# starreeze/drin

Measured on AMD Instinct MI355X. Metric: mention x candidate pairs scored/sec, higher is better.
Workload: dtype bf16x3; 1 GPU; wikimel-shaped scoring forward: 100-cand (+1 answer slot), D=768, R=2048, L=128, P=49, T=64 token-level entity text; parallelism=dp1 (mentions sharded, no collective)

## Files before the change

drin_amd/csrc/entity_cache.hip:

```cpp
#include <string.h>

#include "fused.h"
#include "internal.h"
#include "layout.h"
#include "row_ops.h"

namespace drin {

static inline bool cache_mixed(const drin_config& c) { return c.cache_format == DRIN_CACHE_MIXED_F16; }
static inline size_t cache_row_floats(const drin_config& c) {
  const size_t D = (size_t)c.embed_dim, R = (size_t)c.image_dim;
  return cache_mixed(c) ? 4 * D + R / 2 + 4 : 5 * D + R + 4;
}
constexpr int64_t kCacheSlab = 262144;

struct CacheBuildArgs {
  const float* entity_text;
  const int64_t* entity_mask;
  const float* entity_object;
  const float* entity_object_score;
  float* xt;
  float* cache;
  int64_t ldc, rows;
  int D4, R4, T, Ke;
// ... 410 lines not shown
  }
  __syncthreads();
  float* out1 = a.c_part + (b * a.chunks + blockIdx.x) * (int64_t)(2 * D + 4);
  float* out2 = a.s2_part + (b * a.chunks + blockIdx.x) * (int64_t)(2 * D);
  auto waves_sum = [&](int i) {
    return ((ld4(l_acc + i * 4) + ld4(l_acc + 3 * D + i * 4)) + ld4(l_acc + 6 * D + i * 4)) + ld4(l_acc + 9 * D + i * 4);
  };
  for (int i = threadIdx.x; i < 2 * D4; i += 256) {
    st4(out1 + i * 4, waves_sum(i));
    st4(out2 + i * 4, i < D4 ? waves_sum(2 * D4 + i) : make_float4(0.f, 0.f, 0.f, 0.f));
  }
  if (threadIdx.x < 4) {
    const float* s4 = l_small + 8 + threadIdx.x;
    out1[2 * D + threadIdx.x] = ((s4[0] + s4[4]) + s4[8]) + s4[12];
  }
}

__global__ void __launch_bounds__(256) k_mention_layer1_cached(const float* __restrict__ part, const float* __restrict__ hm,
                                                               int ldhm, const float* __restrict__ cb_t,
                                                               const float* __restrict__ cb_i, const float* __restrict__ b_h,
                                                               float* __restrict__ out, int B, int D, int chunks, float inv_n) {
  const int64_t b = blockIdx.y;
  const int d = blockIdx.x * 256 + threadIdx.x;
  if (d >= D) return;
  const int width = 2 * D + 4;
  float at = 0.f, ai = 0.f, s0 = 0.f, s1 = 0.f, s2 = 0.f, s3 = 0.f;
  for (int c = 0; c < chunks; ++c) {
    const float* p = part + (b * chunks + c) * (int64_t)width;
    at += p[d];
    ai += p[D + d];
    s0 += p[2 * D];
    s1 += p[2 * D + 1];
    s2 += p[2 * D + 2];
    s3 += p[2 * D + 3];
  }
  const float bh = b_h[d], wt = cb_t[d] - bh, wi = cb_i[d] - bh;
  out[b * D + d] = (at + s0 * wt + s1 * wi) * inv_n + hm[b * ldhm + d] + bh;
  out[((int64_t)B + b) * D + d] = (ai + s2 * wt + s3 * wi) * inv_n + hm[((int64_t)B + b) * ldhm + d] + bh;
}

static int cached_chunk_candidates(const drin_config& c) {
  const bool exact = c.embed_dim == 768 && c.image_dim == 2048 && vertex_act(&c) == DRIN_ACT_GELU;
  if (!exact) return 16;
  return c.batch >= 2048 ? 128 : 64;
}

struct CachedLayout {
  size_t span_mean, mimg, vm0, hmfu, e1m, c_part, s2_part, vm1, hm2, agg2, mt2, et1, p_et1, h2, splitk, splitk_floats, total;
  int chunks;
  void build(const drin_config& c) {
    const size_t B = c.batch, N = c.num_candidates, D = c.embed_dim, R = c.image_dim, M = B * N;
    chunks = (int)((N + cached_chunk_candidates(c) - 1) / cached_chunk_candidates(c));
    size_t off = 0;
// ... 276 lines not shown
      DRIN_TRY((launch_cached_pairs_t<3, 8, true, false, true>(a, st)));
    else
      DRIN_TRY((launch_cached_pairs_t<3, 8, false, false, true>(a, st)));
  } else if (a.act_v != DRIN_ACT_GELU && a.D4 <= 64 && a.R4 <= 64)
    DRIN_TRY((launch_cached_pairs_t<1, 1, false, true>(a, st)));
  else if (a.act_v != DRIN_ACT_GELU)
    DRIN_TRY((launch_cached_pairs_t<3, 8, false, true>(a, st)));
  else if (a.D4 <= 64 && a.R4 <= 64)
    DRIN_TRY((launch_cached_pairs_t<1, 1, false>(a, st)));
  else if (a.D4 == 192 && a.R4 == 512)
    DRIN_TRY((launch_cached_pairs_t<3, 8, true>(a, st)));
  else
    DRIN_TRY((launch_cached_pairs_t<3, 8, false>(a, st)));

  float* vm1 = ws + L.vm1;
  {
    KernelTimer timer(DRIN_KC_GCN, st);
    hipLaunchKernelGGL(k_mention_layer1_cached, dim3((unsigned)cdiv(D, 256), (unsigned)B), dim3(256), 0, st, ws + L.c_part,
                       hmfu, 2 * D, pb + P.cb_t, pb + P.cb_i, L1.b_h, vm1, B, D, L.chunks, 1.0f / (float)N);
    DRIN_CHECK_LAUNCH("k_mention_layer1_cached");
  }
  DRIN_TRY(run_folded_mention_finish(cfg, params, pb, P, weight_planes, vm1, ws + L.hm2, msk, st));
  return run_folded_tail(cfg, params, pb, P, L.chunks, ws + L.s2_part, vm1, ws + L.agg2, ws + L.mt2, ws + L.hm2, ws + L.e1m, ws + L.h2,
                         planes ? nullptr : ws + L.et1, planes ? e1_hi : nullptr, weight_planes, msk, {}, scores, st);
}

}
```

drin_amd/csrc/fused.h:

```cpp
#pragma once
#include <hip/hip_runtime.h>
#include <stddef.h>
#include <stdint.h>
#include <string.h>

#include "../../include/drin_hip.h"
#include "layout.h"

namespace drin {

struct Prepared {
  size_t wcat1, bcat1, ecat, etmp, k_t, k_i, c_txt, c_img, cb_t, cb_i, total;
  size_t p_ctxt, p_cimg, p_wh2;
  size_t p_wmt, p_wmi, p_wcat1, p_ecat, p_wet, p_wei, p_wh1;
  size_t p_cimg_f16;
  size_t cimg_f16_scale;
  void build(const drin_config& c) {
    const size_t D = c.embed_dim, R = c.image_dim;
    size_t off = 0;
    auto take = [&off](size_t n) {
      const size_t o = off;
      off += (n + 63) & ~(size_t)63;
      return o;
    };
    wcat1 = take(2 * D * D);
    bcat1 = take(2 * D);
    ecat = take(D * (D + R));
    etmp = take(D * (D + R));
    k_t = take(D);
    k_i = take(D);
    c_txt = take(D * D);
    c_img = take(D * R);
    cb_t = take(D);
    cb_i = take(D);
    p_ctxt = take(D * D);
    p_cimg = take(D * R);
    p_wh2 = take(D * D);
    p_wmt = take(D * D);
    p_wmi = take(D * R);
    p_wcat1 = take(2 * D * D);
    p_ecat = take(D * (D + R));
    p_wet = take(D * D);
    p_wei = take(D * R);
    p_wh1 = take(D * D);
    p_cimg_f16 = take(D * R / 2 + 2);
    cimg_f16_scale = take(2);
    total = off;
  }
};

int fused_supported(const drin_config* c);
int cached_chunks_per_mention(const drin_config& c);

struct StreamArgs {
  const void* entity_text;
  const int64_t* entity_mask;
  const void* entity_image;
  const void* entity_object;
  const float* entity_object_score;
// ... 6 lines not shown
  const void* mobj;
  const float* mscore;
  const float* fu;
  const float* q;
  const float* k_t;
  const float* k_i;
  float* xt_out;
  void* xt_hi;
  void* xt_lo;
  void* xi_hi;
  void* xi_lo;
  float* xi_scale;
  void* xi_f16;
  float* e0m;
  float* e1m;
  float* s_part;
  float* s_text;
  float* s_img;
  float* sig;
  int B, N, D4, R4, T, Km, Ke, chunks, ldq, ldfu, dynamic, bf16_features;
  int act_e;
  float mask[4];
  float cos_eps, miei_eps, clip;
};

struct PairArgs {
  const float* h_text;
  const float* h_image;
  const float* hm;
  const float* c_t;
  const float* c_i;
  const float* gamma;
  const float* beta;
  const float* e0m;
  const float* e1m;
  float* et1;
  void* et1_hi;
  void* et1_lo;
  float* s2_part;
  int B, N, D4, chunks, ldhm;
  int act_v;
  float ln_eps;
};

struct FinalArgs {
  const float* h2;
  const float* hm2;
  const float* b_h2;
  const float* gamma;
  const float* beta;
  const float* e1m;
  const float* mt2;
  float* scores;
  int B, N, D4, chunks;
// ... 10 lines not shown
}
template <class Args>
void set_vertex_fields(Args& a, const drin_config& c) {
  a.ln_eps = c.layer_norm_eps, a.act_v = vertex_act(&c);
}
template <class Args>
void set_edge_fields(Args& a, const drin_config& c) {
  a.R4 = c.image_dim / 4;
  a.Km = c.mention_objects;
  a.dynamic = c.dynamic_edges != 0;
  a.act_e = edge_act(&c);
  for (int k = 0; k < 4; ++k) a.mask[k] = c.edge_enabled[k];
  a.cos_eps = c.cosine_eps, a.miei_eps = c.miei_eps, a.clip = c.clip_scale;
}

size_t entity_stream_lds_bytes(const StreamArgs& a);
int launch_entity_stream(const StreamArgs& a, hipStream_t st);
int launch_reduce_stream_partials(const float* part, float* s_text, float* s_img, float* sig, int B, int D, int R,
                                  int chunks, hipStream_t st);
int launch_mention_input1(const float* T, const float* T2, const float* sig, const float* b_et, const float* b_ei,
                          const float* v0, float* out, int B, int D, int N, hipStream_t st);
int launch_pair_layer1(const PairArgs& a, hipStream_t st);
int launch_mention_input2(const float* part, const float* mt1, float* out, int B, int D, int N, int chunks,
                          hipStream_t st);
int launch_pair_final(const FinalArgs& a, hipStream_t st);

struct GemmScratch {
  float* p = nullptr;
  size_t floats = 0;
};
int run_folded_head(const drin_config* cfg, const drin_batch* b, const drin_params* params, const float* prepared, const Prepared& P,
                    bool weight_planes, float* span_mean, float* mimg, float* vm0, float* hmfu, GemmScratch mention_sk, hipStream_t st);
int run_folded_mention_finish(const drin_config* cfg, const drin_params* params, const float* prepared, const Prepared& P,
                              bool weight_planes, float* vm1, float* hm2, GemmScratch mention_sk, hipStream_t st);
int run_folded_tail(const drin_config* cfg, const drin_params* params, const float* prepared, const Prepared& P, int chunks,
                    const float* s2_part, const float* vm1, float* agg2, float* mt2, const float* hm2, const float* e1m, float* h2,
// ... 4 lines not shown
```

drin_amd/csrc/fused_forward.hip:

```cpp
#include <string.h>

#include "fused.h"
#include "internal.h"
#include "layout.h"

namespace drin {

constexpr int kMixedMinCandidates = 64;

struct FusedLayout {
  size_t span_mean, mimg, vm0, hmfu, q, e0m, e1m, xt, s_part, s_text, s_img, sig, tm, tm2, agg1, vm1, hm2, h_text, h_image,
      et1, s2_part, agg2, mt2, p_xt, p_xi, p_et1, xi_scale, splitk, splitk_floats, pair_splitk, pair_splitk_floats, total;
  int chunks;
  void build(const drin_config& c) {
    const size_t B = c.batch, N = c.num_candidates, D = c.embed_dim, R = c.image_dim, M = B * N;
    chunks = (int)(B >= 2048 ? (N + 127) / 128 : B >= 1024 ? (N + 47) / 48 : (N + 15) / 16);
    size_t off = 0;
    auto take = [&off](size_t n) {
      const size_t o = off;
      off += (n + 63) & ~(size_t)63;
      return o;
    };
    span_mean = take(B * D);
    mimg = take(B * R);
    vm0 = take(2 * B * D);
    hmfu = take(2 * B * 2 * D);
    q = take(2 * B * (D + R));
    e0m = take(4 * M);
    e1m = take(4 * M);
    xt = take(c.entity_tokens > 0 ? M * D : 0);
    s_part = take(B * chunks * (2 * D + 2 * R + 4));
    s_text = take(2 * B * D);
    s_img = take(2 * B * R);
    sig = take(4 * B);
    tm = take(2 * B * D);
    tm2 = take(2 * B * D);
    agg1 = take(2 * B * D);
    vm1 = take(2 * B * D);
    hm2 = take(2 * B * D);
    h_text = take(M * D);
    h_image = take(M * D);
    et1 = take(M * D);
    s2_part = take(B * chunks * 2 * D);
    agg2 = take(B * D);
    mt2 = take(B * D);
    const bool planes = c.precision == DRIN_PREC_BF16X3 || c.precision == DRIN_PREC_BF16X3_ALL || c.precision == DRIN_PREC_BF16X3_IF16;
    p_xt = take(planes ? M * D : 0);
    p_xi = take(!planes ? 0 : c.num_entities > 0 ? M * R : c.precision == DRIN_PREC_BF16X3_IF16 ? M * R / 2 : 0);
    p_et1 = take(planes ? M * D : 0);
    xi_scale = take(c.precision == DRIN_PREC_BF16X3_IF16 ? M : 0);
    splitk_floats = 2 * B <= 512 ? 8 * 2 * B * (D + R) : 0;
    if (planes && splitk_floats < (size_t)192 * 65536) splitk_floats = (size_t)192 * 65536;
// ... 120 lines not shown
  DRIN_TRY(launch_gemm_nn(L1.w_h, D, params->w_entity_text, D, pb + P.c_txt, D, D, D, D, false, F32, st));
  DRIN_TRY(launch_gemm_nn(L1.w_h, D, params->w_entity_image, R, pb + P.c_img, R, D, R, D, false, F32, st));
  DRIN_TRY(launch_gemm_nt(params->b_entity_text, D, L1.w_h, D, L1.b_h, pb + P.cb_t, D, 1, D, D, false, F32, st));
  DRIN_TRY(launch_gemm_nt(params->b_entity_image, D, L1.w_h, D, L1.b_h, pb + P.cb_i, D, 1, D, D, false, F32, st));
  {
    const size_t dd = (size_t)D * D, dr = (size_t)D * R;
    __bf16* q = reinterpret_cast<__bf16*>(pb + P.p_ctxt);
    DRIN_TRY(launch_split_planes(pb + P.c_txt, q, q + dd, dd, st));
    q = reinterpret_cast<__bf16*>(pb + P.p_cimg);
    DRIN_TRY(launch_split_planes(pb + P.c_img, q, q + dr, dr, st));
    DRIN_TRY(launch_to_f16_scaled(pb + P.c_img, pb + P.p_cimg_f16, (int64_t)dr, pb + P.cimg_f16_scale, st));
    q = reinterpret_cast<__bf16*>(pb + P.p_wh2);
    DRIN_TRY(launch_split_planes(params->layer[1].w_h, q, q + dd, dd, st));
    struct { size_t off; const float* w; size_t n; } extra[] = {
        {P.p_wmt, params->w_mention_text, dd},  {P.p_wmi, params->w_mention_image, dr},
        {P.p_wcat1, pb + P.wcat1, 2 * dd},      {P.p_ecat, pb + P.ecat, dd + dr},
        {P.p_wet, params->w_entity_text, dd},   {P.p_wei, params->w_entity_image, dr},
        {P.p_wh1, L1.w_h, dd}};
    for (const auto& e : extra) {
      q = reinterpret_cast<__bf16*>(pb + e.off);
      DRIN_TRY(launch_split_planes(e.w, q, q + e.n, e.n, st));
    }
  }
  return DRIN_OK;
}

}

namespace drin {

static int folded_precision(const drin_config* c) { return c->precision == DRIN_PREC_BF16X3_IF16 ? (int)DRIN_PREC_BF16X3 : c->precision; }

int run_folded_head(const drin_config* cfg, const drin_batch* b, const drin_params* params, const float* pb, const Prepared& P,
// ... 131 lines not shown
  sa.k_t = pb + P.k_t;
  sa.k_i = pb + P.k_i;
  sa.xt_out = planes ? nullptr : ws + L.xt;
  if (planes) {
    sa.xt_hi = xt_hi;
    sa.xt_lo = xt_exact ? nullptr : xt_hi + MD;
    if (xi_planes) {
      sa.xi_hi = xi_hi;
      sa.xi_lo = bf16_feat ? nullptr : xi_hi + MR;
    }
  }
  sa.xi_scale = if16 ? ws + L.xi_scale : nullptr;
  sa.xi_f16 = if16 ? static_cast<void*>(xi_hi) : nullptr;
  sa.e0m = ws + L.e0m;
  sa.e1m = ws + L.e1m;
  sa.s_part = ws + L.s_part;
  sa.T = cfg->entity_tokens;
  sa.Ke = cfg->entity_objects;
  sa.chunks = L.chunks;
  sa.bf16_features = bf16_feat ? 1 : 0;
  sa.s_text = ws + L.s_text;
  sa.s_img = ws + L.s_img;
  sa.sig = ws + L.sig;
  DRIN_TRY(launch_entity_stream(sa, st));
  if (L.chunks > 1)
    DRIN_TRY(launch_reduce_stream_partials(ws + L.s_part, ws + L.s_text, ws + L.s_img, ws + L.sig, B, D, R, L.chunks, st));
  DRIN_TRY(launch_gemm_nt_pair({ws + L.s_text, params->w_entity_text, nullptr, ws + L.tm, D, D, D, 2 * (int64_t)B, D, D, wp(P.p_wet)},
                               {ws + L.s_img, params->w_entity_image, nullptr, ws + L.tm2, R, R, D, 2 * (int64_t)B, D, R,
                                wp(P.p_wei)},
                               prec, st, msk.p, msk.floats));
  DRIN_TRY(launch_mention_input1(ws + L.tm, ws + L.tm2, ws + L.sig, params->b_entity_text, params->b_entity_image, vm0, ws + L.agg1, B, D, N, st));
  float* vm1 = ws + L.vm1;
  DRIN_TRY(launch_gemm_nt(ws + L.agg1, D, L1.w_h, D, L1.b_h, vm1, D, 2 * (int64_t)B, D, D, false, prec, st, msk.p, msk.floats, wp(P.p_wh1)));
  DRIN_TRY(run_folded_mention_finish(cfg, params, pb, P, planes, vm1, ws + L.hm2, msk, st));
  const GemmScratch psk = L.pair_splitk_floats ? GemmScratch{ws + L.pair_splitk, L.pair_splitk_floats} : msk;
  if (planes) {
    const __bf16* ct = reinterpret_cast<const __bf16*>(pb + P.p_ctxt);
    const __bf16* ci = reinterpret_cast<const __bf16*>(pb + P.p_cimg);
    DRIN_TRY(launch_gemm_x3_planes(xt_hi, xt_exact ? nullptr : xt_hi + MD, D, ct, ct + (size_t)D * D, D, nullptr, ws + L.h_text, D, M, D,
                                   D, st, psk.p, psk.floats));
    if (if16)
      DRIN_TRY(launch_gemm_f16_planes(xi_hi, R, pb + P.p_cimg_f16, R, ws + L.xi_scale, pb + P.cimg_f16_scale, ws + L.h_image, D, M, D, R,
                                      st, psk.p, psk.floats));
    else if (xi_planes)
      DRIN_TRY(launch_gemm_x3_planes(xi_hi, bf16_feat ? nullptr : xi_hi + MR, R, ci, ci + (size_t)D * R, R, nullptr, ws + L.h_image, D, M,
                                     D, R, st, psk.p, psk.floats));
    else if (bf16_feat)
      DRIN_TRY(launch_gemm_x3_planes(b->entity_image, nullptr, R, ci, ci + (size_t)D * R, R, nullptr, ws + L.h_image, D, M, D, R, st, psk.p,
                                     psk.floats));
// ... 11 lines not shown
  pa.h_image = ws + L.h_image;
  pa.hm = hmfu;
  pa.ldhm = 2 * D;
  pa.c_t = pb + P.cb_t;
  pa.c_i = pb + P.cb_i;
  pa.gamma = L1.ln_weight;
  pa.beta = L1.ln_bias;
  pa.e0m = ws + L.e0m;
  pa.e1m = ws + L.e1m;
  pa.et1 = planes ? nullptr : ws + L.et1;
  if (planes) {
    pa.et1_hi = e1_hi;
    pa.et1_lo = e1_hi + MD;
  }
  pa.s2_part = ws + L.s2_part;
  pa.chunks = L.chunks;
  DRIN_TRY(launch_pair_layer1(pa, st));
  return run_folded_tail(cfg, params, pb, P, L.chunks, ws + L.s2_part, vm1, ws + L.agg2, ws + L.mt2, ws + L.hm2, ws + L.e1m, ws + L.h_text,
                         planes ? nullptr : ws + L.et1, planes ? e1_hi : nullptr, planes, msk, psk, scores, st);
}

}

extern "C" {

int32_t drin_workgroups_per_mention(const drin_config* cfg, int32_t cached) {
  if (validate_config(cfg) != DRIN_OK || fused_supported(cfg) != DRIN_OK) return 0;
  if (cached) return cached_chunks_per_mention(*cfg);
  FusedLayout L;
  L.build(*cfg);
  return L.chunks;
}
// ... 56 lines not shown
```

drin_amd/csrc/fused_kernels.hip:

```cpp
#include "device_utils.h"
#include "fused.h"
#include "internal.h"
#include "row_ops.h"

namespace drin {

template <int DV, int RV, bool TOKENS, bool EXACT, typename FT, bool XSCALE = false>
__global__ void __launch_bounds__(256, 2) k_entity_stream(const StreamArgs a) {
  extern __shared__ __attribute__((aligned(16))) float lds[];
  const FT* const f_text = static_cast<const FT*>(a.entity_text);
  const FT* const f_image = static_cast<const FT*>(a.entity_image);
  const FT* const f_object = static_cast<const FT*>(a.entity_object);
  const FT* const f_mobj = static_cast<const FT*>(a.mobj);
  const int D4 = EXACT ? DV * 64 : a.D4, R4 = EXACT ? RV * 64 : a.R4, D = D4 * 4, R = R4 * 4;
  constexpr bool RP = sizeof(FT) == 2 && (RV % 2) == 0;
  auto load_r = [&](const FT* row) -> Row<RV> {
    if constexpr (RP)
      return load_row_stream_pair<RV>(row, (int)(threadIdx.x & 63), R4);
    else
      return load_row_stream<RV>(row, (int)(threadIdx.x & 63), R4);
  };
  float* l_mobj = lds;
  float* l_q = l_mobj + a.Km * R;
  float* l_red = l_q + 2 * R;
  float* l_mt = l_red + 2 * D + 2 * R;
  float* l_small = l_mt + 3 * D;
  const int wave = threadIdx.x >> 6, lane = threadIdx.x & 63;
  const int64_t b = blockIdx.y;
  const int per = (a.N + a.chunks - 1) / a.chunks;
  const int n_begin = blockIdx.x * per, n_end = min(a.N, n_begin + per);
  const bool dyn = a.dynamic != 0;

  for (int i = threadIdx.x; i < a.Km * R4; i += 256) st4(l_mobj + i * 4, ld4(f_mobj + (b * a.Km) * R + i * 4));
  for (int i = threadIdx.x; i < D4; i += 256) st4(l_mt + i * 4, ld4(a.span_mean + b * D + i * 4));
  if (dyn) {
    for (int i = threadIdx.x; i < 2 * R4; i += 256) {
      const int which = i / R4, c4 = i - which * R4;
      st4(l_q + i * 4, ld4(a.q + ((int64_t)which * a.B + b) * a.ldq + D + c4 * 4));
    }
    for (int i = threadIdx.x; i < 2 * D4; i += 256) {
// ... 16 lines not shown
    const Row<DV> m_t = load_row<DV>(l_mt, lane, D4);
    m_t_norm = fmaxf(sqrtf(wave_sum(dot_rows<DV>(m_t, m_t))), a.cos_eps);
  }
  float kap_tt = 0.f, kap_ti = 0.f, kap_it = 0.f, kap_ii = 0.f;
  if (dyn) {
    const Row<DV> fu_t = load_row<DV>(a.fu + b * a.ldfu, lane, D4);
    const Row<DV> fu_i = load_row<DV>(a.fu + ((int64_t)a.B + b) * a.ldfu, lane, D4);
    const Row<DV> k_t = load_row<DV>(a.k_t, lane, D4), k_i = load_row<DV>(a.k_i, lane, D4);
    kap_tt = wave_sum(dot_rows<DV>(fu_t, k_t));
    kap_ti = wave_sum(dot_rows<DV>(fu_t, k_i));
    kap_it = wave_sum(dot_rows<DV>(fu_i, k_t));
    kap_ii = wave_sum(dot_rows<DV>(fu_i, k_i));
  }
  __syncthreads();

  Row<DV> S_tt = zero_row<DV>(), S_it = zero_row<DV>();
  Row<RV> S_ti = zero_row<RV>(), S_ii = zero_row<RV>();
  float sg_tt = 0.f, sg_ti = 0.f, sg_it = 0.f, sg_ii = 0.f;
  const float inv_d = 1.0f / (float)D;

  for (int n = n_begin + wave; n < n_end; n += 4) {
    const int64_t p = b * a.N + n;
    int64_t e = p;
    if (a.entity_index) {
      const int64_t raw = a.entity_index[p];
      e = raw < 0 ? 0 : (raw >= a.num_entities ? a.num_entities - 1 : raw);
      if (e != raw && lane == 0) report_bad_index(a.index_status, p, raw);
    }
    Row<DV> xt;
    float tt;
    if (TOKENS) {
      const int T = a.T;
      int cnt = 0;
      for (int t = lane; t < T; t += 64) cnt += (int)a.entity_mask[e * T + t];
      cnt = (int)wave_sum((float)cnt);
      int stop = cnt - 1;
      if (stop < 0) stop += T;
      stop = stop < 0 ? 0 : (stop > T ? T : stop);
      const FT* base = f_text + e * (int64_t)T * D;
      constexpr bool FLAT = sizeof(FT) == 2 && EXACT && DV == 3;
      const Row<DV> cls = load_row_stream<DV>(base, lane, D4);
      Row<DV> acc = zero_row<DV>();
      int t = 1;
      if constexpr (FLAT) {
        float f0[8], f1[8], f2[8];
#pragma unroll
        for (int i = 0; i < 8; ++i) f0[i] = f1[i] = f2[i] = 0.f;
        const char* flat = reinterpret_cast<const char*>(base) + (size_t)lane * 16;
        auto add8 = [](float (&f)[8], const u32x4_t v) {
#pragma unroll
          for (int i = 0; i < 4; ++i) {
            f[2 * i] += __builtin_bit_cast(float, v[i] << 16);
            f[2 * i + 1] += __builtin_bit_cast(float, v[i] & 0xffff0000u);
          }
        };
// ... 5 lines not shown
            for (int k = 0; k < 3; ++k) r[u][k] = ld16_stream(flat + (size_t)(t + 2 * u) * (2 * 768) + k * 1024);
#pragma unroll
          for (int u = 0; u < 4; ++u) {
            add8(f0, r[u][0]);
            add8(f1, r[u][1]);
            add8(f2, r[u][2]);
          }
        }
        for (; t + 2 <= stop; t += 2) {
          const u32x4_t r0 = ld16_stream(flat + (size_t)t * (2 * 768)), r1 = ld16_stream(flat + (size_t)t * (2 * 768) + 1024),
                        r2 = ld16_stream(flat + (size_t)t * (2 * 768) + 2048);
          add8(f0, r0);
          add8(f1, r1);
          add8(f2, r2);
        }
        float* scr = l_red + wave * 768;
#pragma unroll
        for (int i = 0; i < 8; ++i) {
          const float y1 = __shfl_xor(f1[i], 32), y2 = __shfl_xor(f2[i], 32);
          f0[i] += lane < 32 ? y1 : y2;
          f1[i] += y2;
        }
        st4(scr + 8 * lane, make_float4(f0[0], f0[1], f0[2], f0[3]));
        st4(scr + 8 * lane + 4, make_float4(f0[4], f0[5], f0[6], f0[7]));
        if (lane < 32) {
          st4(scr + 512 + 8 * lane, make_float4(f1[0], f1[1], f1[2], f1[3]));
          st4(scr + 512 + 8 * lane + 4, make_float4(f1[4], f1[5], f1[6], f1[7]));
        }
        __builtin_amdgcn_wave_barrier();
#pragma unroll
        for (int j = 0; j < DV; ++j) acc.v[j] = ld4(scr + 4 * (lane + 64 * j));
// ... 72 lines not shown
      n_ti = edge_act_apply(a.act_e, (d_ti + kap_ti) * inv_d + e_ti);
      n_it = edge_act_apply(a.act_e, (d_it + kap_it) * inv_d + e_it);
      n_ii = edge_act_apply(a.act_e, (d_ii + kap_ii) * inv_d + e_ii);
    }
    if (lane == 0) {
      const int64_t M = (int64_t)a.B * a.N;
      a.e0m[p] = e_tt;
      a.e0m[M + p] = e_ti;
      a.e0m[2 * M + p] = e_it;
      a.e0m[3 * M + p] = e_ii;
      a.e1m[p] = n_tt * a.mask[0];
      a.e1m[M + p] = n_ti * a.mask[1];
      a.e1m[2 * M + p] = n_it * a.mask[2];
      a.e1m[3 * M + p] = n_ii * a.mask[3];
    }
    axpy_row<DV>(S_tt, e_tt, xt);
    axpy_row<DV>(S_it, e_it, xt);
    axpy_row<RV>(S_ti, e_ti, xi);
    axpy_row<RV>(S_ii, e_ii, xi);
    sg_tt += e_tt;
    sg_ti += e_ti;
    sg_it += e_it;
    sg_ii += e_ii;
  }

  for (int w = 0; w < 4; ++w) {
    __syncthreads();
    if (wave == w) {
#pragma unroll
      for (int j = 0; j < DV; ++j) {
        const int c4 = lane + 64 * j;
        if (c4 < D4) {
          float* p0 = l_red + c4 * 4;
          float* p1 = l_red + D + c4 * 4;
          st4(p0, w == 0 ? S_tt.v[j] : ld4(p0) + S_tt.v[j]);
          st4(p1, w == 0 ? S_it.v[j] : ld4(p1) + S_it.v[j]);
        }
      }
#pragma unroll
      for (int j = 0; j < RV; ++j) {
        const int c4 = row_col4<RP>(lane, j);
        if (c4 < R4) {
          float* p0 = l_red + 2 * D + c4 * 4;
          float* p1 = l_red + 2 * D + R + c4 * 4;
          st4(p0, w == 0 ? S_ti.v[j] : ld4(p0) + S_ti.v[j]);
          st4(p1, w == 0 ? S_ii.v[j] : ld4(p1) + S_ii.v[j]);
        }
      }
      if (lane == 0) {
        float* s4 = l_small + a.Km;
        s4[0] = (w == 0 ? 0.f : s4[0]) + sg_tt;
        s4[1] = (w == 0 ? 0.f : s4[1]) + sg_ti;
        s4[2] = (w == 0 ? 0.f : s4[2]) + sg_it;
        s4[3] = (w == 0 ? 0.f : s4[3]) + sg_ii;
      }
    }
  }
  __syncthreads();
  if (a.chunks == 1) {
    for (int i = threadIdx.x; i < 2 * D4; i += 256) {
      const int which = i / D4, c4 = i - which * D4;
      st4(a.s_text + ((int64_t)which * a.B + b) * D + c4 * 4, ld4(l_red + i * 4));
    }
    for (int i = threadIdx.x; i < 2 * R4; i += 256) {
      const int which = i / R4, c4 = i - which * R4;
      st4(a.s_img + ((int64_t)which * a.B + b) * R + c4 * 4, ld4(l_red + 2 * D + i * 4));
    }
    if (threadIdx.x < 4) a.sig[(int64_t)threadIdx.x * a.B + b] = l_small[a.Km + threadIdx.x];
    return;
  }
  float* out = a.s_part + (b * a.chunks + blockIdx.x) * (int64_t)(2 * D + 2 * R + 4);
  for (int i = threadIdx.x; i < (2 * D + 2 * R) / 4; i += 256) st4(out + i * 4, ld4(l_red + i * 4));
  if (threadIdx.x < 4) out[2 * D + 2 * R + threadIdx.x] = l_small[a.Km + threadIdx.x];
}

size_t entity_stream_lds_bytes(const StreamArgs& a) {
  const size_t D = (size_t)a.D4 * 4, R = (size_t)a.R4 * 4;
  return sizeof(float) * (a.Km * R + 2 * R + 2 * D + 2 * R + 3 * D + a.Km + 4);
}

template <int DV, int RV, bool TOKENS, bool EXACT, typename FT, bool XSCALE = false>
static int launch_stream_ft(const StreamArgs& a, hipStream_t st) {
  const size_t lds = entity_stream_lds_bytes(a);
  auto kern = k_entity_stream<DV, RV, TOKENS, EXACT, FT, XSCALE>;
  static DynLdsOptIn opt_in;
  if (lds > 48 * 1024)
    DRIN_TRY(ensure_dynamic_lds(opt_in, reinterpret_cast<const void*>(kern), (int)lds, "hipFuncSetAttribute(entity_stream)"));
  KernelTimer timer(DRIN_KC_STREAM, st);
  hipLaunchKernelGGL(kern, dim3((unsigned)a.chunks, (unsigned)a.B), dim3(256), lds, st, a);
  DRIN_CHECK_LAUNCH("k_entity_stream");
  return DRIN_OK;
}

// ... 19 lines not shown
  if (a.B > 65535) {
    set_error("entity_stream: batch %d exceeds the grid limit; split the batch", a.B);
    return DRIN_E_SHAPE;
  }
  const bool tok = a.T > 0;
  if (a.D4 <= 64 && a.R4 <= 64)
    return tok ? launch_stream_t<1, 1, true, false>(a, st) : launch_stream_t<1, 1, false, false>(a, st);
  if (a.D4 == 192 && a.R4 == 512)
    return tok ? launch_stream_t<3, 8, true, true>(a, st) : launch_stream_t<3, 8, false, true>(a, st);
  if (a.D4 <= 192 && a.R4 <= 512)
    return tok ? launch_stream_t<3, 8, true, false>(a, st) : launch_stream_t<3, 8, false, false>(a, st);
  set_error("entity_stream: D=%d R=%d outside the built instantiations", a.D4 * 4, a.R4 * 4);
  return DRIN_E_UNSUPPORTED;
}

__global__ void __launch_bounds__(256) k_reduce_stream_partials(const float* __restrict__ part, float* __restrict__ s_text,
                                                                float* __restrict__ s_img, float* __restrict__ sig,
                                                                int B, int D, int R, int chunks) {
  const int64_t b = blockIdx.y;
  const int width = 2 * D + 2 * R + 4;
  const int i = (blockIdx.x * 256 + threadIdx.x) * 4;
  if (i >= width) return;
  const float* src = part + (b * chunks) * (int64_t)width + i;
  float4 s = make_float4(0.f, 0.f, 0.f, 0.f);
  int c = 0;
  for (; c + 4 <= chunks; c += 4) {
    const float4 v0 = ld4(src + (int64_t)c * width), v1 = ld4(src + (int64_t)(c + 1) * width);
    const float4 v2 = ld4(src + (int64_t)(c + 2) * width), v3 = ld4(src + (int64_t)(c + 3) * width);
    s = (((s + v0) + v1) + v2) + v3;
  }
  for (; c < chunks; ++c) s = s + ld4(src + (int64_t)c * width);
  if (i < D) {
    st4(s_text + b * D + i, s);
  } else if (i < 2 * D) {
    st4(s_text + ((int64_t)B + b) * D + (i - D), s);
  } else if (i < 2 * D + R) {
    st4(s_img + b * R + (i - 2 * D), s);
  } else if (i < 2 * D + 2 * R) {
    st4(s_img + ((int64_t)B + b) * R + (i - 2 * D - R), s);
  } else {
    sig[b] = s.x;
    sig[(int64_t)B + b] = s.y;
    sig[2 * (int64_t)B + b] = s.z;
    sig[3 * (int64_t)B + b] = s.w;
  }
}

int launch_reduce_stream_partials(const float* part, float* s_text, float* s_img, float* sig, int B, int D, int R,
                                  int chunks, hipStream_t st) {
  if (B <= 0) return DRIN_OK;
  KernelTimer timer(DRIN_KC_GCN, st);
  hipLaunchKernelGGL(k_reduce_stream_partials, dim3((unsigned)cdiv((2 * D + 2 * R + 4) / 4, 256), (unsigned)B), dim3(256), 0,
                     st, part, s_text, s_img, sig, B, D, R, chunks);
  DRIN_CHECK_LAUNCH("k_reduce_stream_partials");
  return DRIN_OK;
}

__global__ void __launch_bounds__(256) k_mention_input1(const float* __restrict__ T, const float* __restrict__ T2,
                                                        const float* __restrict__ sig,
                                                        const float* __restrict__ b_et, const float* __restrict__ b_ei,
                                                        const float* __restrict__ v0, float* __restrict__ out, int B,
                                                        int D, float inv_n) {
  const int64_t i = (int64_t)blockIdx.x * 256 + threadIdx.x;
  if (i >= 2 * (int64_t)B * D) return;
  const int d = (int)(i % D);
  const int64_t row = i / D;
  const int t = (int)(row / B);
  const int64_t b = row - (int64_t)t * B;
  const float sa = sig[(int64_t)(t == 0 ? 0 : 2) * B + b], sb = sig[(int64_t)(t == 0 ? 1 : 3) * B + b];
  out[i] = ((T[i] + T2[i]) + sa * b_et[d] + sb * b_ei[d]) * inv_n + v0[i];
}

int launch_mention_input1(const float* T, const float* T2, const float* sig, const float* b_et, const float* b_ei,
                          const float* v0, float* out, int B, int D, int N, hipStream_t st) {
  if (B <= 0) return DRIN_OK;
  KernelTimer timer(DRIN_KC_GCN, st);
  hipLaunchKernelGGL(k_mention_input1, dim3((unsigned)cdiv(2 * (int64_t)B * D, 256)), dim3(256), 0, st, T, T2, sig,
                     b_et, b_ei, v0, out, B, D, 1.0f / (float)N);
  DRIN_CHECK_LAUNCH("k_mention_input1");
  return DRIN_OK;
}

__global__ void __launch_bounds__(256) k_transpose(const float* __restrict__ in, float* __restrict__ out, int rows,
                                                   int cols) {
  __shared__ float tile[32][33];
  const int tx = threadIdx.x & 31, ty = threadIdx.x >> 5;
  const int r0 = blockIdx.y * 32, c0 = blockIdx.x * 32;
  for (int i = ty; i < 32; i += 8)
    if (r0 + i < rows && c0 + tx < cols) tile[i][tx] = in[(int64_t)(r0 + i) * cols + c0 + tx];
  __syncthreads();
  for (int i = ty; i < 32; i += 8)
    if (c0 + i < cols && r0 + tx < rows) out[(int64_t)(c0 + i) * rows + r0 + tx] = tile[tx][i];
}

// ... 15 lines not shown
  const int64_t b = blockIdx.y;
  const int64_t M = (int64_t)a.B * a.N;
  const int per = (a.N + a.chunks - 1) / a.chunks;
  const int n_begin = blockIdx.x * per, n_end = min(a.N, n_begin + per);
  constexpr int LD = DV * 256;
  {
    const float* src[6] = {a.hm + b * a.ldhm, a.hm + ((int64_t)a.B + b) * a.ldhm, a.c_t, a.c_i, a.gamma, a.beta};
#pragma unroll
    for (int v = 0; v < 6; ++v)
      for (int i = threadIdx.x; i < D4; i += 256) st4(l_const + v * LD + i * 4, ld4(src[v] + i * 4));
  }
  __syncthreads();
  const float *l_hm_t = l_const, *l_hm_i = l_const + LD, *l_ct = l_const + 2 * LD, *l_ci = l_const + 3 * LD;
  const float *l_gamma = l_const + 4 * LD, *l_beta = l_const + 5 * LD;
  Row<DV> S_t = zero_row<DV>(), S_i = zero_row<DV>();
  for (int n = n_begin + wave; n < n_end; n += 4) {
    const int64_t p = b * a.N + n;
    const Row<DV> ht = load_row_stream<DV>(a.h_text + p * D, lane, D4);
    const Row<DV> hi = load_row_stream<DV>(a.h_image + p * D, lane, D4);
    const float e_tt = a.e0m[p], e_ti = a.e0m[M + p], e_it = a.e0m[2 * M + p], e_ii = a.e0m[3 * M + p];
    const Row<DV> et1 = ln_gelu_row_lds<DV, GENERIC_ACT>(combine_rows_lds<DV>(ht, e_tt, l_hm_t, e_it, l_hm_i, l_ct, lane, D4),
                                                         l_gamma, l_beta, lane, D4, a.ln_eps, a.act_v);
    if (a.et1) store_row<DV>(a.et1 + p * D, et1, lane, D4);
    if (a.et1_hi) store_row_planes<DV>(a.et1_hi, a.et1_lo, p * D, et1, lane, D4);
    axpy_row_pk<DV>(S_t, a.e1m[p], et1);
    const Row<DV> ei1 = ln_gelu_row_lds<DV, GENERIC_ACT>(combine_rows_lds<DV>(hi, e_ti, l_hm_t, e_ii, l_hm_i, l_ci, lane, D4),
                                                         l_gamma, l_beta, lane, D4, a.ln_eps, a.act_v);
    axpy_row_pk<DV>(S_i, a.e1m[M + p], ei1);
  }
  for (int w = 0; w < 4; ++w) {
    __syncthreads();
    if (wave == w) {
#pragma unroll
      for (int j = 0; j < DV; ++j) {
        float* p0 = l_red + (j * 64 + lane) * 4;
        float* p1 = l_red + DV * 256 + (j * 64 + lane) * 4;
        st4(p0, w == 0 ? S_t.v[j] : ld4(p0) + S_t.v[j]);
        st4(p1, w == 0 ? S_i.v[j] : ld4(p1) + S_i.v[j]);
      }
    }
  }
  __syncthreads();
  float* out = a.s2_part + (b * a.chunks + blockIdx.x) * (int64_t)(2 * D);
  for (int i = threadIdx.x; i < 2 * D4; i += 256) {
    const int which = i / D4, c4 = i - which * D4;
    st4(out + which * D + c4 * 4, ld4(l_red + which * DV * 256 + c4 * 4));
  }
}

int launch_pair_layer1(const PairArgs& a, hipStream_t st) {
  if (a.B <= 0) return DRIN_OK;
  KernelTimer timer(DRIN_KC_GCN, st);
  if (a.act_v != DRIN_ACT_GELU && a.D4 <= 64)
    hipLaunchKernelGGL((k_pair_layer1<1, false, true>), dim3((unsigned)a.chunks, (unsigned)a.B), dim3(256), 0, st, a);
  else if (a.act_v != DRIN_ACT_GELU && a.D4 <= 192)
    hipLaunchKernelGGL((k_pair_layer1<3, false, true>), dim3((unsigned)a.chunks, (unsigned)a.B), dim3(256), 0, st, a);
  else if (a.D4 <= 64)
    hipLaunchKernelGGL((k_pair_layer1<1, false>), dim3((unsigned)a.chunks, (unsigned)a.B), dim3(256), 0, st, a);
  else if (a.D4 == 192)
    hipLaunchKernelGGL((k_pair_layer1<3, true>), dim3((unsigned)a.chunks, (unsigned)a.B), dim3(256), 0, st, a);
  else if (a.D4 < 192)
    hipLaunchKernelGGL((k_pair_layer1<3, false>), dim3((unsigned)a.chunks, (unsigned)a.B), dim3(256), 0, st, a);
// ... 86 lines not shown
```

Measured before the change: 25.22 million pairs/s.

## Fold entity layer-1 mention aggregation into pair kernel via projected rows

Moves the layer-1 mention aggregation off the raw-feature path: the entity stream kernel no longer accumulates weighted text/image feature sums (including R-wide image rows). Instead the pair kernel accumulates attention-weighted projected rows h_text/h_image into a new partial buffer, and a small mention_layer1 kernel combines them with hm and the folded biases. This drops the partial-reduce kernel, two GEMMs (entity text/image projections to mention space), the mention_input1 kernel, the w_h GEMM and their plane preparation. In exchange the pair kernel does extra axpys and a second block reduction, and the mention finish now runs after the pair kernel instead of before it.

```diff
diff --git a/drin_amd/csrc/entity_cache.hip b/drin_amd/csrc/entity_cache.hip
--- a/drin_amd/csrc/entity_cache.hip
+++ b/drin_amd/csrc/entity_cache.hip
@@ -448,29 +448,6 @@
     const float* s4 = l_small + 8 + threadIdx.x;
     out1[2 * D + threadIdx.x] = ((s4[0] + s4[4]) + s4[8]) + s4[12];
   }
-}
-
-__global__ void __launch_bounds__(256) k_mention_layer1_cached(const float* __restrict__ part, const float* __restrict__ hm,
-                                                               int ldhm, const float* __restrict__ cb_t,
-                                                               const float* __restrict__ cb_i, const float* __restrict__ b_h,
-                                                               float* __restrict__ out, int B, int D, int chunks, float inv_n) {
-  const int64_t b = blockIdx.y;
-  const int d = blockIdx.x * 256 + threadIdx.x;
-  if (d >= D) return;
-  const int width = 2 * D + 4;
-  float at = 0.f, ai = 0.f, s0 = 0.f, s1 = 0.f, s2 = 0.f, s3 = 0.f;
-  for (int c = 0; c < chunks; ++c) {
-    const float* p = part + (b * chunks + c) * (int64_t)width;
-    at += p[d];
-    ai += p[D + d];
-    s0 += p[2 * D];
-    s1 += p[2 * D + 1];
-    s2 += p[2 * D + 2];
-    s3 += p[2 * D + 3];
-  }
-  const float bh = b_h[d], wt = cb_t[d] - bh, wi = cb_i[d] - bh;
-  out[b * D + d] = (at + s0 * wt + s1 * wi) * inv_n + hm[b * ldhm + d] + bh;
-  out[((int64_t)B + b) * D + d] = (ai + s2 * wt + s3 * wi) * inv_n + hm[((int64_t)B + b) * ldhm + d] + bh;
 }
 
 static int cached_chunk_candidates(const drin_config& c) {
@@ -777,12 +754,7 @@
     DRIN_TRY((launch_cached_pairs_t<3, 8, false>(a, st)));
 
   float* vm1 = ws + L.vm1;
-  {
-    KernelTimer timer(DRIN_KC_GCN, st);
-    hipLaunchKernelGGL(k_mention_layer1_cached, dim3((unsigned)cdiv(D, 256), (unsigned)B), dim3(256), 0, st, ws + L.c_part,
-                       hmfu, 2 * D, pb + P.cb_t, pb + P.cb_i, L1.b_h, vm1, B, D, L.chunks, 1.0f / (float)N);
-    DRIN_CHECK_LAUNCH("k_mention_layer1_cached");
-  }
+  DRIN_TRY(launch_mention_layer1(ws + L.c_part, hmfu, 2 * D, pb + P.cb_t, pb + P.cb_i, L1.b_h, vm1, B, D, N, L.chunks, st));
   DRIN_TRY(run_folded_mention_finish(cfg, params, pb, P, weight_planes, vm1, ws + L.hm2, msk, st));
   return run_folded_tail(cfg, params, pb, P, L.chunks, ws + L.s2_part, vm1, ws + L.agg2, ws + L.mt2, ws + L.hm2, ws + L.e1m, ws + L.h2,
                          planes ? nullptr : ws + L.et1, planes ? e1_hi : nullptr, weight_planes, msk, {}, scores, st);
diff --git a/drin_amd/csrc/fused.h b/drin_amd/csrc/fused.h
--- a/drin_amd/csrc/fused.h
+++ b/drin_amd/csrc/fused.h
@@ -12,7 +12,7 @@
 struct Prepared {
   size_t wcat1, bcat1, ecat, etmp, k_t, k_i, c_txt, c_img, cb_t, cb_i, total;
   size_t p_ctxt, p_cimg, p_wh2;
-  size_t p_wmt, p_wmi, p_wcat1, p_ecat, p_wet, p_wei, p_wh1;
+  size_t p_wmt, p_wmi, p_wcat1, p_ecat;
   size_t p_cimg_f16;
   size_t cimg_f16_scale;
   void build(const drin_config& c) {
@@ -40,9 +40,6 @@
     p_wmi = take(D * R);
     p_wcat1 = take(2 * D * D);
     p_ecat = take(D * (D + R));
-    p_wet = take(D * D);
-    p_wei = take(D * R);
-    p_wh1 = take(D * D);
     p_cimg_f16 = take(D * R / 2 + 2);
     cimg_f16_scale = take(2);
     total = off;
@@ -79,10 +76,7 @@
   void* xi_f16;
   float* e0m;
   float* e1m;
-  float* s_part;
-  float* s_text;
-  float* s_img;
-  float* sig;
+  float* m1_part;
   int B, N, D4, R4, T, Km, Ke, chunks, ldq, ldfu, dynamic, bf16_features;
   int act_e;
   float mask[4];
@@ -103,6 +97,7 @@
   void* et1_hi;
   void* et1_lo;
   float* s2_part;
+  float* m1_part;
   int B, N, D4, chunks, ldhm;
   int act_v;
   float ln_eps;
@@ -143,12 +138,12 @@
   a.cos_eps = c.cosine_eps, a.miei_eps = c.miei_eps, a.clip = c.clip_scale;
 }
 
+constexpr bool stream_flat_walk(bool tokens, bool bf16_features, bool exact_widths) { return tokens && bf16_features && exact_widths; }
+constexpr int kStreamFlatScratch = 4 * 768;
 size_t entity_stream_lds_bytes(const StreamArgs& a);
 int launch_entity_stream(const StreamArgs& a, hipStream_t st);
-int launch_reduce_stream_partials(const float* part, float* s_text, float* s_img, float* sig, int B, int D, int R,
-                                  int chunks, hipStream_t st);
-int launch_mention_input1(const float* T, const float* T2, const float* sig, const float* b_et, const float* b_ei,
-                          const float* v0, float* out, int B, int D, int N, hipStream_t st);
+int launch_mention_layer1(const float* part, const float* hm, int ldhm, const float* cb_t, const float* cb_i, const float* b_h,
+                          float* out, int B, int D, int N, int chunks, hipStream_t st);
 int launch_pair_layer1(const PairArgs& a, hipStream_t st);
 int launch_mention_input2(const float* part, const float* mt1, float* out, int B, int D, int N, int chunks,
                           hipStream_t st);
diff --git a/drin_amd/csrc/fused_forward.hip b/drin_amd/csrc/fused_forward.hip
--- a/drin_amd/csrc/fused_forward.hip
+++ b/drin_amd/csrc/fused_forward.hip
@@ -9,7 +9,7 @@
 constexpr int kMixedMinCandidates = 64;
 
 struct FusedLayout {
-  size_t span_mean, mimg, vm0, hmfu, q, e0m, e1m, xt, s_part, s_text, s_img, sig, tm, tm2, agg1, vm1, hm2, h_text, h_image,
+  size_t span_mean, mimg, vm0, hmfu, q, e0m, e1m, xt, m1_part, vm1, hm2, h_text, h_image,
       et1, s2_part, agg2, mt2, p_xt, p_xi, p_et1, xi_scale, splitk, splitk_floats, pair_splitk, pair_splitk_floats, total;
   int chunks;
   void build(const drin_config& c) {
@@ -29,13 +29,7 @@
     e0m = take(4 * M);
     e1m = take(4 * M);
     xt = take(c.entity_tokens > 0 ? M * D : 0);
-    s_part = take(B * chunks * (2 * D + 2 * R + 4));
-    s_text = take(2 * B * D);
-    s_img = take(2 * B * R);
-    sig = take(4 * B);
-    tm = take(2 * B * D);
-    tm2 = take(2 * B * D);
-    agg1 = take(2 * B * D);
+    m1_part = take(B * chunks * (2 * D + 4));
     vm1 = take(2 * B * D);
     hm2 = take(2 * B * D);
     h_text = take(M * D);
@@ -186,9 +180,7 @@
     DRIN_TRY(launch_split_planes(params->layer[1].w_h, q, q + dd, dd, st));
     struct { size_t off; const float* w; size_t n; } extra[] = {
         {P.p_wmt, params->w_mention_text, dd},  {P.p_wmi, params->w_mention_image, dr},
-        {P.p_wcat1, pb + P.wcat1, 2 * dd},      {P.p_ecat, pb + P.ecat, dd + dr},
-        {P.p_wet, params->w_entity_text, dd},   {P.p_wei, params->w_entity_image, dr},
-        {P.p_wh1, L1.w_h, dd}};
+        {P.p_wcat1, pb + P.wcat1, 2 * dd},      {P.p_ecat, pb + P.ecat, dd + dr}};
     for (const auto& e : extra) {
       q = reinterpret_cast<__bf16*>(pb + e.off);
       DRIN_TRY(launch_split_planes(e.w, q, q + e.n, e.n, st));
@@ -350,25 +342,12 @@
   sa.xi_f16 = if16 ? static_cast<void*>(xi_hi) : nullptr;
   sa.e0m = ws + L.e0m;
   sa.e1m = ws + L.e1m;
-  sa.s_part = ws + L.s_part;
+  sa.m1_part = ws + L.m1_part;
   sa.T = cfg->entity_tokens;
   sa.Ke = cfg->entity_objects;
   sa.chunks = L.chunks;
   sa.bf16_features = bf16_feat ? 1 : 0;
-  sa.s_text = ws + L.s_text;
-  sa.s_img = ws + L.s_img;
-  sa.sig = ws + L.sig;
   DRIN_TRY(launch_entity_stream(sa, st));
-  if (L.chunks > 1)
-    DRIN_TRY(launch_reduce_stream_partials(ws + L.s_part, ws + L.s_text, ws + L.s_img, ws + L.sig, B, D, R, L.chunks, st));
-  DRIN_TRY(launch_gemm_nt_pair({ws + L.s_text, params->w_entity_text, nullptr, ws + L.tm, D, D, D, 2 * (int64_t)B, D, D, wp(P.p_wet)},
-                               {ws + L.s_img, params->w_entity_image, nullptr, ws + L.tm2, R, R, D, 2 * (int64_t)B, D, R,
-                                wp(P.p_wei)},
-                               prec, st, msk.p, msk.floats));
-  DRIN_TRY(launch_mention_input1(ws + L.tm, ws + L.tm2, ws + L.sig, params->b_entity_text, params->b_entity_image, vm0, ws + L.agg1, B, D, N, st));
-  float* vm1 = ws + L.vm1;
-  DRIN_TRY(launch_gemm_nt(ws + L.agg1, D, L1.w_h, D, L1.b_h, vm1, D, 2 * (int64_t)B, D, D, false, prec, st, msk.p, msk.floats, wp(P.p_wh1)));
-  DRIN_TRY(run_folded_mention_finish(cfg, params, pb, P, planes, vm1, ws + L.hm2, msk, st));
   const GemmScratch psk = L.pair_splitk_floats ? GemmScratch{ws + L.pair_splitk, L.pair_splitk_floats} : msk;
   if (planes) {
     const __bf16* ct = reinterpret_cast<const __bf16*>(pb + P.p_ctxt);
@@ -410,8 +389,12 @@
     pa.et1_lo = e1_hi + MD;
   }
   pa.s2_part = ws + L.s2_part;
+  pa.m1_part = ws + L.m1_part;
   pa.chunks = L.chunks;
   DRIN_TRY(launch_pair_layer1(pa, st));
+  float* vm1 = ws + L.vm1;
+  DRIN_TRY(launch_mention_layer1(ws + L.m1_part, hmfu, 2 * D, pb + P.cb_t, pb + P.cb_i, L1.b_h, vm1, B, D, N, L.chunks, st));
+  DRIN_TRY(run_folded_mention_finish(cfg, params, pb, P, planes, vm1, ws + L.hm2, msk, st));
   return run_folded_tail(cfg, params, pb, P, L.chunks, ws + L.s2_part, vm1, ws + L.agg2, ws + L.mt2, ws + L.hm2, ws + L.e1m, ws + L.h_text,
                          planes ? nullptr : ws + L.et1, planes ? e1_hi : nullptr, planes, msk, psk, scores, st);
 }
diff --git a/drin_amd/csrc/fused_kernels.hip b/drin_amd/csrc/fused_kernels.hip
--- a/drin_amd/csrc/fused_kernels.hip
+++ b/drin_amd/csrc/fused_kernels.hip
@@ -13,6 +13,7 @@
   const FT* const f_object = static_cast<const FT*>(a.entity_object);
   const FT* const f_mobj = static_cast<const FT*>(a.mobj);
   const int D4 = EXACT ? DV * 64 : a.D4, R4 = EXACT ? RV * 64 : a.R4, D = D4 * 4, R = R4 * 4;
+  constexpr bool FLAT = stream_flat_walk(TOKENS, sizeof(FT) == 2, EXACT && DV == 3 && RV == 8);
   constexpr bool RP = sizeof(FT) == 2 && (RV % 2) == 0;
   auto load_r = [&](const FT* row) -> Row<RV> {
     if constexpr (RP)
@@ -22,8 +23,8 @@
   };
   float* l_mobj = lds;
   float* l_q = l_mobj + a.Km * R;
-  float* l_red = l_q + 2 * R;
-  float* l_mt = l_red + 2 * D + 2 * R;
+  float* l_scr = l_q + 2 * R;
+  float* l_mt = l_scr + (FLAT ? kStreamFlatScratch : 0);
   float* l_small = l_mt + 3 * D;
   const int wave = threadIdx.x >> 6, lane = threadIdx.x & 63;
   const int64_t b = blockIdx.y;
@@ -70,8 +71,6 @@
   }
   __syncthreads();
 
-  Row<DV> S_tt = zero_row<DV>(), S_it = zero_row<DV>();
-  Row<RV> S_ti = zero_row<RV>(), S_ii = zero_row<RV>();
   float sg_tt = 0.f, sg_ti = 0.f, sg_it = 0.f, sg_ii = 0.f;
   const float inv_d = 1.0f / (float)D;
 
@@ -94,7 +93,6 @@
       if (stop < 0) stop += T;
       stop = stop < 0 ? 0 : (stop > T ? T : stop);
       const FT* base = f_text + e * (int64_t)T * D;
-      constexpr bool FLAT = sizeof(FT) == 2 && EXACT && DV == 3;
       const Row<DV> cls = load_row_stream<DV>(base, lane, D4);
       Row<DV> acc = zero_row<DV>();
       int t = 1;
@@ -130,7 +128,7 @@
           add8(f1, r1);
           add8(f2, r2);
         }
-        float* scr = l_red + wave * 768;
+        float* scr = l_scr + wave * 768;
 #pragma unroll
         for (int i = 0; i < 8; ++i) {
           const float y1 = __shfl_xor(f1[i], 32), y2 = __shfl_xor(f2[i], 32);
@@ -233,69 +231,30 @@
       a.e1m[2 * M + p] = n_it * a.mask[2];
       a.e1m[3 * M + p] = n_ii * a.mask[3];
     }
-    axpy_row<DV>(S_tt, e_tt, xt);
-    axpy_row<DV>(S_it, e_it, xt);
-    axpy_row<RV>(S_ti, e_ti, xi);
-    axpy_row<RV>(S_ii, e_ii, xi);
     sg_tt += e_tt;
     sg_ti += e_ti;
     sg_it += e_it;
     sg_ii += e_ii;
   }
 
-  for (int w = 0; w < 4; ++w) {
-    __syncthreads();
-    if (wave == w) {
-#pragma unroll
-      for (int j = 0; j < DV; ++j) {
-        const int c4 = lane + 64 * j;
-        if (c4 < D4) {
-          float* p0 = l_red + c4 * 4;
-          float* p1 = l_red + D + c4 * 4;
-          st4(p0, w == 0 ? S_tt.v[j] : ld4(p0) + S_tt.v[j]);
-          st4(p1, w == 0 ? S_it.v[j] : ld4(p1) + S_it.v[j]);
-        }
-      }
-#pragma unroll
-      for (int j = 0; j < RV; ++j) {
-        const int c4 = row_col4<RP>(lane, j);
-        if (c4 < R4) {
-          float* p0 = l_red + 2 * D + c4 * 4;
-          float* p1 = l_red + 2 * D + R + c4 * 4;
-          st4(p0, w == 0 ? S_ti.v[j] : ld4(p0) + S_ti.v[j]);
-          st4(p1, w == 0 ? S_ii.v[j] : ld4(p1) + S_ii.v[j]);
-        }
-      }
-      if (lane == 0) {
-        float* s4 = l_small + a.Km;
-        s4[0] = (w == 0 ? 0.f : s4[0]) + sg_tt;
-        s4[1] = (w == 0 ? 0.f : s4[1]) + sg_ti;
-        s4[2] = (w == 0 ? 0.f : s4[2]) + sg_it;
-        s4[3] = (w == 0 ? 0.f : s4[3]) + sg_ii;
-      }
-    }
+  if (lane == 0) {
+    float* s4 = l_small + a.Km + 4 * wave;
+    s4[0] = sg_tt;
+    s4[1] = sg_ti;
+    s4[2] = sg_it;
+    s4[3] = sg_ii;
   }
   __syncthreads();
-  if (a.chunks == 1) {
-    for (int i = threadIdx.x; i < 2 * D4; i += 256) {
-      const int which = i / D4, c4 = i - which * D4;
-      st4(a.s_text + ((int64_t)which * a.B + b) * D + c4 * 4, ld4(l_red + i * 4));
-    }
-    for (int i = threadIdx.x; i < 2 * R4; i += 256) {
-      const int which = i / R4, c4 = i - which * R4;
-      st4(a.s_img + ((int64_t)which * a.B + b) * R + c4 * 4, ld4(l_red + 2 * D + i * 4));
-    }
-    if (threadIdx.x < 4) a.sig[(int64_t)threadIdx.x * a.B + b] = l_small[a.Km + threadIdx.x];
-    return;
-  }
-  float* out = a.s_part + (b * a.chunks + blockIdx.x) * (int64_t)(2 * D + 2 * R + 4);
-  for (int i = threadIdx.x; i < (2 * D + 2 * R) / 4; i += 256) st4(out + i * 4, ld4(l_red + i * 4));
-  if (threadIdx.x < 4) out[2 * D + 2 * R + threadIdx.x] = l_small[a.Km + threadIdx.x];
+  if (threadIdx.x < 4) {
+    const float* s4 = l_small + a.Km + threadIdx.x;
+    a.m1_part[(b * a.chunks + blockIdx.x) * (int64_t)(2 * D + 4) + 2 * D + threadIdx.x] = ((s4[0] + s4[4]) + s4[8]) + s4[12];
+  }
 }
 
 size_t entity_stream_lds_bytes(const StreamArgs& a) {
   const size_t D = (size_t)a.D4 * 4, R = (size_t)a.R4 * 4;
-  return sizeof(float) * (a.Km * R + 2 * R + 2 * D + 2 * R + 3 * D + a.Km + 4);
+  const bool flat = stream_flat_walk(a.T > 0, a.bf16_features != 0, a.D4 == 192 && a.R4 == 512);
+  return sizeof(float) * (a.Km * R + 2 * R + (flat ? kStreamFlatScratch : 0) + 3 * D + a.Km + 16);
 }
 
 template <int DV, int RV, bool TOKENS, bool EXACT, typename FT, bool XSCALE = false>
@@ -345,70 +304,36 @@
   return DRIN_E_UNSUPPORTED;
 }
 
-__global__ void __launch_bounds__(256) k_reduce_stream_partials(const float* __restrict__ part, float* __restrict__ s_text,
-                                                                float* __restrict__ s_img, float* __restrict__ sig,
-                                                                int B, int D, int R, int chunks) {
+__global__ void __launch_bounds__(256) k_mention_layer1(const float* __restrict__ part, const float* __restrict__ hm,
+                                                        int ldhm, const float* __restrict__ cb_t,
+                                                        const float* __restrict__ cb_i, const float* __restrict__ b_h,
+                                                        float* __restrict__ out, int B, int D, int chunks, float inv_n) {
   const int64_t b = blockIdx.y;
-  const int width = 2 * D + 2 * R + 4;
-  const int i = (blockIdx.x * 256 + threadIdx.x) * 4;
-  if (i >= width) return;
-  const float* src = part + (b * chunks) * (int64_t)width + i;
-  float4 s = make_float4(0.f, 0.f, 0.f, 0.f);
-  int c = 0;
-  for (; c + 4 <= chunks; c += 4) {
-    const float4 v0 = ld4(src + (int64_t)c * width), v1 = ld4(src + (int64_t)(c + 1) * width);
-    const float4 v2 = ld4(src + (int64_t)(c + 2) * width), v3 = ld4(src + (int64_t)(c + 3) * width);
-    s = (((s + v0) + v1) + v2) + v3;
-  }
-  for (; c < chunks; ++c) s = s + ld4(src + (int64_t)c * width);
-  if (i < D) {
-    st4(s_text + b * D + i, s);
-  } else if (i < 2 * D) {
-    st4(s_text + ((int64_t)B + b) * D + (i - D), s);
-  } else if (i < 2 * D + R) {
-    st4(s_img + b * R + (i - 2 * D), s);
-  } else if (i < 2 * D + 2 * R) {
-    st4(s_img + ((int64_t)B + b) * R + (i - 2 * D - R), s);
-  } else {
-    sig[b] = s.x;
-    sig[(int64_t)B + b] = s.y;
-    sig[2 * (int64_t)B + b] = s.z;
-    sig[3 * (int64_t)B + b] = s.w;
-  }
-}
-
-int launch_reduce_stream_partials(const float* part, float* s_text, float* s_img, float* sig, int B, int D, int R,
-                                  int chunks, hipStream_t st) {
+  const int d = blockIdx.x * 256 + threadIdx.x;
+  if (d >= D) return;
+  const int width = 2 * D + 4;
+  float at = 0.f, ai = 0.f, s0 = 0.f, s1 = 0.f, s2 = 0.f, s3 = 0.f;
+  for (int c = 0; c < chunks; ++c) {
+    const float* p = part + (b * chunks + c) * (int64_t)width;
+    at += p[d];
+    ai += p[D + d];
+    s0 += p[2 * D];
+    s1 += p[2 * D + 1];
+    s2 += p[2 * D + 2];
+    s3 += p[2 * D + 3];
+  }
+  const float bh = b_h[d], wt = cb_t[d] - bh, wi = cb_i[d] - bh;
+  out[b * D + d] = (at + s0 * wt + s1 * wi) * inv_n + hm[b * ldhm + d] + bh;
+  out[((int64_t)B + b) * D + d] = (ai + s2 * wt + s3 * wi) * inv_n + hm[((int64_t)B + b) * ldhm + d] + bh;
+}
+
+int launch_mention_layer1(const float* part, const float* hm, int ldhm, const float* cb_t, const float* cb_i, const float* b_h,
+                          float* out, int B, int D, int N, int chunks, hipStream_t st) {
   if (B <= 0) return DRIN_OK;
   KernelTimer timer(DRIN_KC_GCN, st);
-  hipLaunchKernelGGL(k_reduce_stream_partials, dim3((unsigned)cdiv((2 * D + 2 * R + 4) / 4, 256), (unsigned)B), dim3(256), 0,
-                     st, part, s_text, s_img, sig, B, D, R, chunks);
-  DRIN_CHECK_LAUNCH("k_reduce_stream_partials");
-  return DRIN_OK;
-}
-
-__global__ void __launch_bounds__(256) k_mention_input1(const float* __restrict__ T, const float* __restrict__ T2,
-                                                        const float* __restrict__ sig,
-                                                        const float* __restrict__ b_et, const float* __restrict__ b_ei,
-                                                        const float* __restrict__ v0, float* __restrict__ out, int B,
-                                                        int D, float inv_n) {
-  const int64_t i = (int64_t)blockIdx.x * 256 + threadIdx.x;
-  if (i >= 2 * (int64_t)B * D) return;
-  const int d = (int)(i % D);
-  const int64_t row = i / D;
-  const int t = (int)(row / B);
-  const int64_t b = row - (int64_t)t * B;
-  const float sa = sig[(int64_t)(t == 0 ? 0 : 2) * B + b], sb = sig[(int64_t)(t == 0 ? 1 : 3) * B + b];
-  out[i] = ((T[i] + T2[i]) + sa * b_et[d] + sb * b_ei[d]) * inv_n + v0[i];
-}
-
-int launch_mention_input1(const float* T, const float* T2, const float* sig, const float* b_et, const float* b_ei,
-                          const float* v0, float* out, int B, int D, int N, hipStream_t st) {
-  if (B <= 0) return DRIN_OK;
-  KernelTimer timer(DRIN_KC_GCN, st);
-  hipLaunchKernelGGL(k_mention_input1, dim3((unsigned)cdiv(2 * (int64_t)B * D, 256)), dim3(256), 0, st, T, T2, sig,
-                     b_et, b_ei, v0, out, B, D, 1.0f / (float)N);
-  DRIN_CHECK_LAUNCH("k_mention_input1");
+  hipLaunchKernelGGL(k_mention_layer1, dim3((unsigned)cdiv(D, 256), (unsigned)B), dim3(256), 0, st, part, hm, ldhm, cb_t, cb_i, b_h,
+                     out, B, D, chunks, 1.0f / (float)N);
+  DRIN_CHECK_LAUNCH("k_mention_layer1");
   return DRIN_OK;
 }
 
@@ -454,11 +379,17 @@
   const float *l_hm_t = l_const, *l_hm_i = l_const + LD, *l_ct = l_const + 2 * LD, *l_ci = l_const + 3 * LD;
   const float *l_gamma = l_const + 4 * LD, *l_beta = l_const + 5 * LD;
   Row<DV> S_t = zero_row<DV>(), S_i = zero_row<DV>();
+  Row<DV> A_t = zero_row<DV>(), A_i = zero_row<DV>();
   for (int n = n_begin + wave; n < n_end; n += 4) {
+    asm volatile("" ::: "memory");
     const int64_t p = b * a.N + n;
     const Row<DV> ht = load_row_stream<DV>(a.h_text + p * D, lane, D4);
     const Row<DV> hi = load_row_stream<DV>(a.h_image + p * D, lane, D4);
     const float e_tt = a.e0m[p], e_ti = a.e0m[M + p], e_it = a.e0m[2 * M + p], e_ii = a.e0m[3 * M + p];
+    axpy_row_pk<DV>(A_t, e_tt, ht);
+    axpy_row_pk<DV>(A_t, e_ti, hi);
+    axpy_row_pk<DV>(A_i, e_it, ht);
+    axpy_row_pk<DV>(A_i, e_ii, hi);
     const Row<DV> et1 = ln_gelu_row_lds<DV, GENERIC_ACT>(combine_rows_lds<DV>(ht, e_tt, l_hm_t, e_it, l_hm_i, l_ct, lane, D4),
                                                          l_gamma, l_beta, lane, D4, a.ln_eps, a.act_v);
     if (a.et1) store_row<DV>(a.et1 + p * D, et1, lane, D4);
@@ -468,24 +399,27 @@
                                                          l_gamma, l_beta, lane, D4, a.ln_eps, a.act_v);
     axpy_row_pk<DV>(S_i, a.e1m[M + p], ei1);
   }
-  for (int w = 0; w < 4; ++w) {
+  auto reduce_store = [&](const Row<DV>& r0, const Row<DV>& r1, float* out) {
+    for (int w = 0; w < 4; ++w) {
+      __syncthreads();
+      if (wave == w) {
+#pragma unroll
+        for (int j = 0; j < DV; ++j) {
+          float* p0 = l_red + (j * 64 + lane) * 4;
+          float* p1 = l_red + DV * 256 + (j * 64 + lane) * 4;
+          st4(p0, w == 0 ? r0.v[j] : ld4(p0) + r0.v[j]);
+          st4(p1, w == 0 ? r1.v[j] : ld4(p1) + r1.v[j]);
+        }
+      }
+    }
     __syncthreads();
-    if (wave == w) {
-#pragma unroll
-      for (int j = 0; j < DV; ++j) {
-        float* p0 = l_red + (j * 64 + lane) * 4;
-        float* p1 = l_red + DV * 256 + (j * 64 + lane) * 4;
-        st4(p0, w == 0 ? S_t.v[j] : ld4(p0) + S_t.v[j]);
-        st4(p1, w == 0 ? S_i.v[j] : ld4(p1) + S_i.v[j]);
-      }
-    }
-  }
-  __syncthreads();
-  float* out = a.s2_part + (b * a.chunks + blockIdx.x) * (int64_t)(2 * D);
-  for (int i = threadIdx.x; i < 2 * D4; i += 256) {
-    const int which = i / D4, c4 = i - which * D4;
-    st4(out + which * D + c4 * 4, ld4(l_red + which * DV * 256 + c4 * 4));
-  }
+    for (int i = threadIdx.x; i < 2 * D4; i += 256) {
+      const int which = i / D4, c4 = i - which * D4;
+      st4(out + which * D + c4 * 4, ld4(l_red + which * DV * 256 + c4 * 4));
+    }
+  };
+  reduce_store(S_t, S_i, a.s2_part + (b * a.chunks + blockIdx.x) * (int64_t)(2 * D));
+  reduce_store(A_t, A_i, a.m1_part + (b * a.chunks + blockIdx.x) * (int64_t)(2 * D + 4));
 }
 
 int launch_pair_layer1(const PairArgs& a, hipStream_t st) {
```

Result: faster. 25.82 million pairs/s, median of 6 (+2.4%).
